# rvp-group/srrg2_laser_slam_2d

Hardware: AMD Instinct MI355X
Metric: scan-to-map alignments/sec (1081-beam vs 100k-pt map, 20 GN iters) (higher is better)
Workload: dtype f32

## Files before the change

### srrg2_laser_slam_2d_amd/csrc/lsm2d_capi_aligner.inc

```
extern "C" uint64_t lsm2d_pair_hash(uint32_t slice, uint32_t fixed_idx, uint32_t moving_idx) {
  const uint32_t a = fixed_idx * 0x9E3779B1u, b = (moving_idx ^ (slice * 0x632BE5ABu)) * 0x85EBCA77u;
  uint32_t lo = a ^ ((b << 13) | (b >> 19)), hi = b ^ ((a << 19) | (a >> 13));
  lo += ((lo << 17) | (lo >> 15)) ^ b;
  hi += ((hi << 11) | (hi >> 21)) ^ a;
  return ((uint64_t) hi << 32) | (uint64_t) lo;
}

extern "C" int32_t lsm2d_stats_capacity(const lsm2d_aligner_params* ap) {
  if (!ap) return 1;
  const long long c = (long long) (ap->max_iterations > 0 ? ap->max_iterations : 0) * (ap->enable_inlier_only_runs ? 2 : 1);
  return (int32_t) (c < 1 ? 1 : (c > 0x7fffffff ? 0x7fffffff : c));
}

struct lsm2d_pending {
  lsm2d_context* ctx = nullptr;
  Lane* lane = nullptr;
  size_t o_pose = 0, o_H = 0, o_status = 0, o_its = 0, o_stats = 0, o_last_pose = 0, o_clock = 0, o_cand = 0;
  int n = 0, stats_stride = 0, n_clock = 0, clock_stride = 0;
  bool zero_copy = false, want_stats = false, want_last_pose = false, stamps = false, timed = false, async = false;
};
static int align_batch_finish(lsm2d_pending& P, float* out_pose, float* out_H, int32_t* out_status, int32_t* out_its, lsm2d_iteration_stats* out_stats, float* out_last_pose);

static constexpr int kEmptyBatch = 0x7e7e7e7e;

// ... 571 lines not shown
    if (zero_copy) { const unsigned long long epoch = ctx->sync_epoch; we = wait_for_statuses(ctx, (const int32_t*) (hs + o_status), n, L.ev_done); ctx->sync_epoch = epoch; }
    else we = hipEventSynchronize(L.ev_done);
    L.busy = false;
    if (ctx->inflight > 0) --ctx->inflight;
    HIPCHK(ctx, we);
  }
  else if (zero_copy) HIPCHK(ctx, wait_for_statuses(ctx, (const int32_t*) (hs + o_status), n));
  else HIPCHK(ctx, stream_sync(ctx));
  ctx->timed_lane = (int) (&L - ctx->lanes); ctx->have_timing = P.timed;
  {
    static_assert(kStatusNotWritten == -1, "the memsets above write 0xFF bytes");
    const int32_t* st = (const int32_t*) (hs + o_status);
    for (int i = 0; i < n; ++i) if (st[i] == kStatusNotWritten) { for (Lane& any : ctx->lanes) any.order_valid = false; return fail(ctx, LSM2D_DEVICE_ERROR, "align_batch: an alignment's workgroup never reported (placement or launch fault)"); }
  }
  memcpy(out_pose, hs + o_pose, sizeof(float) * 3 * (size_t) n);
  if (out_H) memcpy(out_H, hs + o_H, sizeof(float) * 9 * (size_t) n);
  memcpy(out_status, hs + o_status, sizeof(int32_t) * (size_t) n);
  if (out_its) memcpy(out_its, hs + o_its, sizeof(int32_t) * (size_t) n);
  if (out_stats) memcpy(out_stats, hs + o_stats, sizeof(StatsDev) * (size_t) n * (size_t) stats_stride);
  if (out_last_pose) memcpy(out_last_pose, hs + o_last_pose, sizeof(float) * 3 * (size_t) n);
  if (P.want_stats) {
    const uint32_t* cw = (const uint32_t*) (hs + P.o_cand);
    long long its = 0, builds = 0, over = 0;
    for (int i = 0; i < n; ++i) { its += cw[i] & 0xFFFFu; builds += (cw[i] >> 16) & 0xFFu; over += cw[i] >> 24; }
    ctx->last_cand_iterations = (int) std::min(its, (long long) 0x7fffffff); ctx->last_cand_builds = (int) std::min(builds, (long long) 0x7fffffff); ctx->last_cand_overflows = (int) std::min(over, (long long) 0x7fffffff);
  }
  if (stamps) {
    const unsigned long long* ck = (const unsigned long long*) (hs + o_clock);
    std::vector<double> khz; std::vector<unsigned long long> life;
    for (int i = 0; i < n_clock; ++i) if (ck[4 * i + 1] > 0) { khz.push_back((double) ck[4 * i] / (double) ck[4 * i + 1] * 1e5); life.push_back(ck[4 * i + 1] * 10ull); }
    if (const char* dump = getenv("LSM2D_DUMP_STAMPS")) {
      if (FILE* f = fopen(dump, "a")) {
        unsigned long long t0 = ~0ull; for (int i = 0; i < n_clock; ++i) if (ck[4 * i + 1] > 0 && ck[4 * i + 2] < t0) t0 = ck[4 * i + 2];
        fprintf(f, "# launch n=%d stride=%d\n", n, clock_stride);
        for (int i = 0; i < n_clock; ++i)
          fprintf(f, "%d %llu %llu %llu 0x%llx\n", i * clock_stride, ck[4 * i], ck[4 * i + 1], ck[4 * i + 2] - t0, ck[4 * i + 3]);
        fclose(f);
      }
    }
    if (!khz.empty()) {
      std::nth_element(khz.begin(), khz.begin() + khz.size() / 2, khz.end()); ctx->last_clock_khz = (long long) khz[khz.size() / 2];
      std::nth_element(life.begin(), life.begin() + life.size() / 2, life.end()); ctx->last_wg_lifetime_ns = (long long) life[life.size() / 2];
    }
  }
  return LSM2D_SUCCESS;
}

extern "C" int lsm2d_align_batch(lsm2d_context* ctx, const lsm2d_aligner_params* ap, const lsm2d_batch* b, float* out_pose,
                                 float* out_H, int32_t* out_status, int32_t* out_its, lsm2d_iteration_stats* out_stats) {
  return align_batch_impl(ctx, ap, b, out_pose, out_H, out_status, out_its, out_stats, nullptr);
}

extern "C" int lsm2d_align_batch_begin(lsm2d_context* ctx, const lsm2d_aligner_params* ap, const lsm2d_batch* b, int32_t want_stats, lsm2d_pending** out_pending) {
  if (!ctx || !out_pending) return fail(ctx, LSM2D_BAD_ARGUMENT, "align_batch_begin: null argument");
  *out_pending = nullptr;
  lsm2d_pending* P = new (std::nothrow) lsm2d_pending;
  if (!P) return LSM2D_OUT_OF_MEMORY;
  static float dummy_pose; static int32_t dummy_status; static lsm2d_iteration_stats dummy_stats;
  const int rc = align_batch_impl(ctx, ap, b, &dummy_pose, nullptr, &dummy_status, nullptr, want_stats ? &dummy_stats : nullptr, nullptr, nullptr, P);
  if (rc != LSM2D_SUCCESS || !P->ctx) { const bool empty = rc == LSM2D_SUCCESS; delete P; if (!empty) return rc; P = new (std::nothrow) lsm2d_pending; if (!P) return LSM2D_OUT_OF_MEMORY; }
  *out_pending = P;
  return LSM2D_SUCCESS;
}
extern "C" int lsm2d_align_batch_wait(lsm2d_pending* pending, float* out_pose, float* out_H, int32_t* out_status, int32_t* out_its, lsm2d_iteration_stats* out_stats) {
  if (!pending) return LSM2D_BAD_ARGUMENT;
  if (!pending->ctx) { delete pending; return LSM2D_SUCCESS; }
  lsm2d_context* ctx = pending->ctx;
// ... 80 lines not shown
```

### srrg2_laser_slam_2d_amd/csrc/lsm2d_device.h

```cpp
#pragma once
#include <hip/hip_runtime.h>
#include <stdint.h>

namespace lsm2d {

typedef unsigned long long u64;
static constexpr u64 kEmptyCell = ~0ull;

#define LSM2D_DEV __device__ __forceinline__
#define LSM2D_HD  __host__ __device__ inline

struct Iso { float c, s, tx, ty; };

struct ProjK {
  float K00, K01;
  float rmin, rmax;
  float r2lo, r2hi;
  float colsf;
  int   cols;
  int   tiny_ok;
};

LSM2D_HD void sincos_fixed(float x, float& sn, float& cs) {
  const float kf = __builtin_rintf(x * 6.3661974669e-01f);
// ... 259 lines not shown
    const int g = code & 511, t0 = (code >> 9) * B;
    const int nsteps = T_steps - t0 < B ? T_steps - t0 : B;
    const int voff = g * (int) sizeof(float4) + t0 * row_bytes;
    int idx = 2 * (g * T_steps + t0);
    auto load = [&](int soff) {
      const u32x4 w = __builtin_amdgcn_raw_buffer_load_b128(rsrc, voff, soff, 0);
      return make_float4(__uint_as_float(w.x), __uint_as_float(w.y), __uint_as_float(w.z), __uint_as_float(w.w));
    };
    auto pair = [&](const float4& v, int i) {
      project_point_stream<kGuarded>(T, P, v.x, v.y, i, canvas);
      project_point_stream<kGuarded>(T, P, v.z, v.w, i + 1, canvas);
    };
    int t = 0, soff = 0;
    float4 va = load(0);
    for (; t + 2 <= nsteps; t += 2) {
      const float4 vb = load(soff + row_bytes);
      pair(va, idx);
      soff += 2 * row_bytes;
      va = load(soff);
      pair(vb, idx + 2);
      idx += 4;
    }
    if (t < nsteps) pair(va, idx);
  }
}
template <int kStride = 0>
LSM2D_DEV void project_cloud_list(const float4* __restrict__ lane_xy, int T_steps, const Iso& T, const ProjK& P, u64* canvas, int tid, int nthreads,
                                  const uint16_t* units, int n_units, int B) {
  if (P.tiny_ok) project_cloud_list_t<false, kStride>(lane_xy, T_steps, T, P, canvas, tid, nthreads, units, n_units, B);
  else project_cloud_list_t<true, kStride>(lane_xy, T_steps, T, P, canvas, tid, nthreads, units, n_units, B);
}

LSM2D_DEV float cand_depth_margin(float r, float m_t, float tn2 ) { return m_t + __builtin_fmaf(1.0e-6f, r, __builtin_fmaf(2.6e-7f, tn2, 1e-7f)); }
template <bool kGuarded>
LSM2D_DEV int cand_classify(const Iso& T, const ProjK& P, float px, float py, float m_t, float m_th, float tn2, float& r, float& md, int& col) {
  r = 0.0f; md = 0.0f; col = -1;
  if (!(__builtin_fabsf(px) < __builtin_huge_valf() && __builtin_fabsf(py) < __builtin_huge_valf())) return 0;
  float qx, qy;
  xf_point(T, px, py, qx, qy);
  const float r2 = __builtin_fmaf(qx, qx, qy * qy);
  if (!(r2 >= 1e-30f && r2 <= 1e37f)) return 1;
  float y0;
  r = sqrt_rn_seed(r2, y0);
  md = cand_depth_margin(r, m_t, tn2);
  if (r < P.rmin - md || r > P.rmax + md) return 0;
  if (!(md <= 0.25f * r)) return 1;
  const float th = bearing<kGuarded>(qy, qx, r, y0);
  const float u = __builtin_fmaf(P.K00, th, P.K01);
  const float aK = __builtin_fabsf(P.K00);
  const float cs = __builtin_fmaf(aK, __builtin_fmaf(1.06f, md / (r - md), 1.001f * m_th), 4e-3f);
  if ((3.14159274101257324f - __builtin_fabsf(th)) * aK <= cs) return 1;
  if (u < -cs || u > P.colsf + cs) return 0;
  asm("v_cvt_flr_i32_f32 %0, %1" : "=v"(col) : "v"(u));
  if ((unsigned) col >= (unsigned) P.cols) return 1;
  if (!(r >= P.rmin + md && r <= P.rmax - md)) return 1;
  const float f = u - (float) col;
  return (f > cs && 1.0f - f > cs) ? 2 : 1;
}
template <int kStride, class F>
LSM2D_DEV void cand_for_each_pair(const float4* __restrict__ lane_xy, int T_steps, int tid, int nthreads, const uint16_t* units, int n_units, int B, F f) {
  typedef unsigned u32x4 __attribute__((ext_vector_type(4)));
  const unsigned long long pb = reinterpret_cast<unsigned long long>(lane_xy);
  const unsigned pb_hi = (unsigned) __builtin_amdgcn_readfirstlane((int) (pb >> 32));
  const unsigned pb_lo = (unsigned) __builtin_amdgcn_readfirstlane((int) (unsigned) pb);
  float4* ubase = reinterpret_cast<float4*>(((unsigned long long) pb_hi << 32) | (unsigned long long) pb_lo);
  const __amdgpu_buffer_rsrc_t rsrc = __builtin_amdgcn_make_buffer_rsrc(ubase, (short) 0, 0x7fffffff, 0x00020000);
  const int row_bytes = nthreads * (int) sizeof(float4);
  for (int k = tid; k < n_units; k += kStride) {
    const int code = (int) units[k];
    const int g = code & 511, t0 = (code >> 9) * B;
    const int nsteps = T_steps - t0 < B ? T_steps - t0 : B;
    const int voff = g * (int) sizeof(float4) + t0 * row_bytes;
    int idx = 2 * (g * T_steps + t0);
    for (int t = 0; t < nsteps; ++t, idx += 2) {
      const u32x4 w = __builtin_amdgcn_raw_buffer_load_b128(rsrc, voff + t * row_bytes, 0, 0);
      f(__uint_as_float(w.x), __uint_as_float(w.y), __uint_as_float(w.z), __uint_as_float(w.w), idx);
    }
  }
}
template <bool kGuarded, int kStride>
LSM2D_DEV void cand_blockers_t(const float4* __restrict__ lane_xy, int T_steps, const Iso& Tin, const ProjK& Pin, int tid, int nthreads, const uint16_t* units, int n_units, int B,
                               uint32_t* blk, float m_t, float m_th) {
  const Iso T = Tin; const ProjK P = Pin;
  const float tn2 = __builtin_fabsf(T.tx) + __builtin_fabsf(T.ty) + 2.0f * m_t;
  auto one = [&](float px, float py) {
    float r, md; int col;
    if (cand_classify<kGuarded>(T, P, px, py, m_t, m_th, tn2, r, md, col) == 2) atomicMin(&blk[col], __float_as_uint(r + md));
  };
  cand_for_each_pair<kStride>(lane_xy, T_steps, tid, nthreads, units, n_units, B, [&](float ax, float ay, float bx, float by, int) { one(ax, ay); one(bx, by); });
}
template <bool kGuarded, int kStride>
LSM2D_DEV void cand_collect_t(const float4* __restrict__ lane_xy, int T_steps, const Iso& Tin, const ProjK& Pin, int tid, int nthreads, const uint16_t* units, int n_units, int B,
                              const uint32_t* blk, uint32_t* cand, int cap, int* count, float m_t, float m_th) {
  const Iso T = Tin; const ProjK P = Pin;
  const float tn2 = __builtin_fabsf(T.tx) + __builtin_fabsf(T.ty) + 2.0f * m_t;
  auto keeps = [&](float px, float py) -> bool {
    float r, md; int col;
    const int cl = cand_classify<kGuarded>(T, P, px, py, m_t, m_th, tn2, r, md, col);
    if (cl != 2) return cl == 1;
    return !(__uint_as_float(blk[col]) < r - md);
  };
  cand_for_each_pair<kStride>(lane_xy, T_steps, tid, nthreads, units, n_units, B, [&](float ax, float ay, float bx, float by, int idx) {
    const bool k0 = keeps(ax, ay), k1 = keeps(bx, by);
    const u64 b0 = __ballot(k0), b1 = __ballot(k1);
    const u64 act = b0 | b1;
    if (act) {
      const int n0 = __popcll(b0);
      int base = 0;
      if ((int) __builtin_amdgcn_mbcnt_hi((unsigned) (act >> 32), __builtin_amdgcn_mbcnt_lo((unsigned) act, 0u)) == 0 && (k0 || k1)) base = atomicAdd(count, n0 + __popcll(b1));
      base = __builtin_amdgcn_readlane(base, __builtin_amdgcn_readfirstlane(__builtin_ctzll(act)));
      const int p0 = base + (int) __builtin_amdgcn_mbcnt_hi((unsigned) (b0 >> 32), __builtin_amdgcn_mbcnt_lo((unsigned) b0, 0u));
      const int p1 = base + n0 + (int) __builtin_amdgcn_mbcnt_hi((unsigned) (b1 >> 32), __builtin_amdgcn_mbcnt_lo((unsigned) b1, 0u));
      if (k0 && p0 < cap) cand[p0] = (uint32_t) idx;
      if (k1 && p1 < cap) cand[p1] = (uint32_t) (idx + 1);
    }
  });
}
template <bool kGuarded, int kStride>
LSM2D_DEV void project_candidates_t(const float2* __restrict__ mxy, const Iso& Tin, const ProjK& Pin, u64* canvas, int tid, const uint32_t* cand, int n) {
  const Iso T = Tin; ProjK P = Pin;
  asm volatile("" : "+v"(P.K01));
  int k = tid;
  if (k >= n) return;
  int idx = (int) cand[k];
  float2 p = mxy[idx];
  for (; k < n; k += kStride) {
    const int kn = k + kStride;
    const int idn = (int) cand[kn < n ? kn : k];
    const float2 pn = mxy[idn];
    project_point_stream<kGuarded>(T, P, p.x, p.y, idx, canvas);
    idx = idn; p = pn;
  }
}
LSM2D_HD int cand_blocker_words(int cols) { return (cols + 3) & ~3; }
template <int kStride, int kChunks>
LSM2D_DEV void cand_build(const float4* lane_xy, int T_steps, const Iso& T, const ProjK& P, int tid, const uint16_t* units, int n_units, int B, uint32_t* blk, const int* par, int* count) {
  const int cap = __builtin_amdgcn_readfirstlane(par[1]);
  const float m_t = __int_as_float(__builtin_amdgcn_readfirstlane(par[4])), m_th = __int_as_float(__builtin_amdgcn_readfirstlane(par[5]));
  uint32_t* cand = blk + cand_blocker_words(P.cols);
  for (int c = tid; c < P.cols; c += kStride) blk[c] = 0xFFFFFFFFu;
  __syncthreads();
  if (P.tiny_ok) cand_blockers_t<false, kStride>(lane_xy, T_steps, T, P, tid, kChunks, units, n_units, B, blk, m_t, m_th);
  else cand_blockers_t<true, kStride>(lane_xy, T_steps, T, P, tid, kChunks, units, n_units, B, blk, m_t, m_th);
  __syncthreads();
  if (P.tiny_ok) cand_collect_t<false, kStride>(lane_xy, T_steps, T, P, tid, kChunks, units, n_units, B, blk, cand, cap, count, m_t, m_th);
  else cand_collect_t<true, kStride>(lane_xy, T_steps, T, P, tid, kChunks, units, n_units, B, blk, cand, cap, count, m_t, m_th);
}
LSM2D_DEV bool cand_pose_within(const Iso& N, const Iso& L, float m_t, float m_th) {
  if (__float_as_uint(N.c) == __float_as_uint(L.c) && __float_as_uint(N.s) == __float_as_uint(L.s)) {
    const float ex = N.tx - L.tx, ey = N.ty - L.ty;
    return ex * ex + ey * ey <= m_t * m_t * 0.999999f;
  }
  const float cd = N.c * L.c + N.s * L.s, sd = N.s * L.c - N.c * L.s;
  const float dx = N.tx - (cd * L.tx - sd * L.ty), dy = N.ty - (sd * L.tx + cd * L.ty);
  const float lim = m_t - 4e-7f * (__builtin_fabsf(N.tx) + __builtin_fabsf(N.ty) + __builtin_fabsf(L.tx) + __builtin_fabsf(L.ty));
  return cd > 0.5f && __builtin_fabsf(sd) <= m_th - 3e-7f && lim > 0.0f && dx * dx + dy * dy <= lim * lim * 0.999999f;
}

LSM2D_DEV void project_cloud_units(const float4* __restrict__ lane_xy, int T_steps, const Iso& T, const ProjK& P, u64* canvas, int tid, int nthreads,
                                   const uint16_t* surv, int s, int B, int nb) {
  if (P.tiny_ok) project_cloud_units_t<false>(lane_xy, T_steps, T, P, canvas, tid, nthreads, surv, s, B, nb);
  else project_cloud_units_t<true>(lane_xy, T_steps, T, P, canvas, tid, nthreads, surv, s, B, nb);
}

LSM2D_DEV void project_cloud_lanes(const float4* __restrict__ lane_xy, int T_steps, const Iso& T, const ProjK& P,
                                   u64* canvas, int tid, int nthreads) {
  if (P.tiny_ok) project_cloud_lanes_t<false>(lane_xy, T_steps, T, P, canvas, tid, nthreads);
  else project_cloud_lanes_t<true>(lane_xy, T_steps, T, P, canvas, tid, nthreads);
}

struct Accum {
  float h00, h01, h02, h11, h12, h22, b0, b1, b2, chi_in, chi_out;
  int n_in, n_out, n_corr;
};
LSM2D_DEV void accum_zero(Accum& a) {
  a.h00 = a.h01 = a.h02 = a.h11 = a.h12 = a.h22 = a.b0 = a.b1 = a.b2 = a.chi_in = a.chi_out = 0.0f;
  a.n_in = a.n_out = a.n_corr = 0;
// ... 355 lines not shown
```

### srrg2_laser_slam_2d_amd/csrc/lsm2d_k_align.h

```cpp
template <bool kHasProj, bool kHasNN, bool kHasDist, bool kHasKd = false, int kNNMode = 0, bool kSeq = false, int kW = kAlignBlock, bool kCandLists = false>
LSM2D_DEV void align_body(const AlignArgs& A, int a_given = -1) {
  static_assert(kW == kAlignBlock || (kNNMode == 5 && !kSeq && kW % 64 == 0 && kW >= 256 && kW < kAlignBlock), "narrow workgroups: the culled projective stream only");
  __builtin_assume(A.n_slices >= 1 && A.n_slices <= kMaxSlices);
  constexpr bool kNNGlobal = kNNMode == 1, kNNLds = kNNMode == 2;
  constexpr bool kKdAllLds = kNNMode == 3, kKdTop = kNNMode == 4;
  constexpr bool kProjCulled = kNNMode == 5;
  constexpr bool kCand = kCandLists && kProjCulled && !kSeq && kW == kAlignBlock;
  static_assert(kNNMode == 0 || ((kNNMode <= 2) && kHasNN && !kHasProj && !kHasDist && !kHasKd) || ((kNNMode == 3 || kNNMode == 4) && kHasKd && !kHasProj && !kHasDist && !kHasNN) ||
                (kNNMode == 5 && kHasProj && !kHasNN && !kHasDist && !kHasKd), "kNNMode: one finder only");
  extern __shared__ __align__(16) unsigned char smem[];
  u64* mcan = reinterpret_cast<u64*>(smem);
  u64* fcan = mcan + A.cols_max;
  float* red = reinterpret_cast<float*>(fcan + A.fcan_total + ((A.cols_max + A.fcan_total) & 1));
  float2* l_sxy = reinterpret_cast<float2*>(red + (kAlignBlock / 64) * kAccumWords);
  int* l_qc = reinterpret_cast<int*>(red + (kAlignBlock / 64) * kAccumWords);
  uint16_t* l_cst = reinterpret_cast<uint16_t*>(l_sxy + A.nn_lds_points);
  uint16_t* l_sidx = l_cst + ((A.nn_lds_cells + 2) & ~1);
  float4* l_kpl = reinterpret_cast<float4*>(red + (kAlignBlock / 64) * kAccumWords);
  int2* l_klk = reinterpret_cast<int2*>(l_kpl + A.kd_lds_nodes);
  float2* l_kxy = reinterpret_cast<float2*>(l_klk + A.kd_lds_nodes + (A.kd_lds_nodes & 1));
  float2* l_knr = l_kxy + A.kd_lds_points + (A.kd_lds_points & 1);
  __shared__ float s_pose[3];
  __shared__ Iso   s_iso[kMaxSlices];
  __shared__ float s_H[9], s_sum[kAccumWords + 2];
  constexpr int kSumPairs = 13, kSumActive = 14, kSumWords = 15;
  static_assert(kSumWords <= kAccumWords + 2 && kAccumWords + 2 == 16, "s_sum: one word per lane of a row of sixteen");
  __shared__ int   s_done, s_status, s_last_n_in;
  __shared__ float s_prev_chi;
  __shared__ u64 s_dig;
  __shared__ int s_it0;
  __shared__ int s_phase, s_phase_start, s_phase_end;
  __shared__ uint16_t s_surv[kAlignBlock];
  __shared__ int s_wcnt[2 * (kAlignBlock / 64)];
  __shared__ int s_nunits[kMaxSlices], s_rebuild[kMaxSlices];
  __shared__ Iso s_list_iso[kMaxSlices];
  __shared__ Iso s_cand_iso;
  __shared__ int s_cand_n, s_cand_state, s_cand_stat;
  __shared__ int s_cand_par[6];
  uint16_t* l_units = reinterpret_cast<uint16_t*>(smem + A.units_off);
  float* l_rec = reinterpret_cast<float*>(smem + (kSeq ? A.seq_off : 0));
  __shared__ uint32_t s_ring[3 * kFfRing];
  __shared__ int s_ring_n, s_skip;
  __shared__ uint32_t* s_ff_rows;
  __shared__ PriorDev s_prior;

  const int a = a_given >= 0 ? a_given : (A.order ? __builtin_amdgcn_readfirstlane(A.order[blockIdx.x]) : (int) blockIdx.x), tid = threadIdx.x;
  constexpr int nwaves = kW / 64;
  constexpr int kPriorWords = (int) (sizeof(PriorDev) / sizeof(float));
  __shared__ unsigned long long s_clk[2];
#ifdef LSM2D_PHASE_PROBE
  __shared__ unsigned long long s_ph[4];
  if (tid == 0) { s_ph[0] = s_ph[1] = s_ph[2] = 0; s_ph[3] = __builtin_amdgcn_s_memtime(); }
#define LSM2D_PH_STAMP(k) do { if (tid == 0) { const unsigned long long now__ = __builtin_amdgcn_s_memtime(); s_ph[k] += now__ - s_ph[3]; s_ph[3] = now__; } } while (0)
#if LSM2D_PHASE_PROBE + 0 == 2
#define LSM2D_PH(k) LSM2D_PH_STAMP((k) == 0 ? 1 : (k))
#define LSM2D_PH_LISTS() do { } while (0)
#define LSM2D_PH_STREAM() LSM2D_PH_STAMP(0)
#elif LSM2D_PHASE_PROBE + 0 == 3
#define LSM2D_PH(k) LSM2D_PH_STAMP(2)
#define LSM2D_PH_LISTS() LSM2D_PH_STAMP(0)
#define LSM2D_PH_STREAM() LSM2D_PH_STAMP(1)
#elif LSM2D_PHASE_PROBE + 0 == 4
#define LSM2D_PH(k) do { } while (0)
#define LSM2D_PH_LISTS() do { } while (0)
#define LSM2D_PH_STREAM() LSM2D_PH_STAMP(1)
#define LSM2D_PH_SUMS() LSM2D_PH_STAMP(0)
#define LSM2D_PH_TAIL() LSM2D_PH_STAMP(2)
#else
#define LSM2D_PH(k) LSM2D_PH_STAMP(k)
#define LSM2D_PH_LISTS() do { } while (0)
#define LSM2D_PH_STREAM() do { } while (0)
#endif
#else
#define LSM2D_PH(k) do { } while (0)
#define LSM2D_PH_LISTS() do { } while (0)
#define LSM2D_PH_STREAM() do { } while (0)
#endif
#ifndef LSM2D_PH_SUMS
#define LSM2D_PH_SUMS() do { } while (0)
#define LSM2D_PH_TAIL() do { } while (0)
#endif
  if (A.wg_place && tid == 0) A.wg_place[blockIdx.x] = place_key();
  const bool stamp = A.clock_out && tid == 0 && a % A.clock_stride == 0;
  if (stamp) { s_clk[0] = __builtin_amdgcn_s_memtime(); s_clk[1] = __builtin_amdgcn_s_memrealtime(); }
  if (A.prior && tid >= 64 && tid < 64 + kPriorWords)
    ((float*) &s_prior)[tid - 64] = A.inline_n1 ? ((const float*) &A.prior1)[tid - 64] : ((const float*) (A.prior + a))[tid - 64];

  constexpr int kPqRowWords = 5, kPqOccWords = 128 * kPqRowWords;
  __shared__ unsigned s_pqbb[4];
  __shared__ float s_pq[4];
  const bool pq_on = (kHasNN || kHasKd || kHasDist) && A.pq_cull_off > 0;
  uint32_t* l_occ = reinterpret_cast<uint32_t*>(smem + (pq_on ? A.pq_cull_off : 0));
  u64* l_keep = reinterpret_cast<u64*>(l_occ + kPqOccWords);
  auto ordered = [](float f) { const unsigned u = __float_as_uint(f); return (u & 0x80000000u) ? ~u : (u | 0x80000000u); };
  auto unordered = [](unsigned k) { return __uint_as_float((k & 0x80000000u) ? (k & 0x7FFFFFFFu) : ~k); };
  if (pq_on) {
    for (int i = tid; i < kPqOccWords; i += kAlignBlock) l_occ[i] = 0u;
    if (tid < 4) s_pqbb[tid] = tid < 2 ? 0xFFFFFFFFu : 0u;
  }

  if (kHasProj && !kHasNN && !kHasDist && !kHasKd && A.inline_n1)
    for (int s = 0; s < A.n_slices; ++s) if (A.s[s].unpack_src) unpack_fixed_set(A.s[s], tid, kW);
  for (int i = tid; i < A.fcan_total; i += kW) fcan[i] = kEmptyCell;
  for (int i = tid; i < A.cols_max; i += kW) mcan[i] = kEmptyCell;
  auto begin_iteration = [&]() {
    for (int s = 0; s < A.n_slices; ++s) {
      float Xe[3] = {s_pose[0], s_pose[1], s_pose[2]};
      if (A.s[s].has_sensor) compose(A.s[s].cSinv, A.s[s].sSinv, A.s[s].Sinv, s_pose, Xe);
      sincos_fixed(Xe[2], s_iso[s].s, s_iso[s].c); s_iso[s].tx = Xe[0]; s_iso[s].ty = Xe[1];
    }
    float zf = 0.0f; int zi = 0;
    asm volatile("" : "+v"(zf), "+v"(zi));
    for (int k = 0; k < 11; ++k) s_sum[k] = zf;
// ... 144 lines not shown
        ++acc.n_corr; acc.n_in += inl ? 1 : 0; acc.n_out += inl ? 0 : 1;
        seq_have = true;
      };
      int seq_fill = 0;
      auto seq_walk_buffer = [&](int n) {
        if (tid < ((n + 7) & ~7) - n) { float z[kSeqFields]; seq_zero(z); seq_store(l_rec, n + tid, z); }
        __syncthreads();
        if (tid < 64) seq_acc = seq_walk<LSM2D_SEQ_WALK_PRIO != 0>(l_rec, n, tid, seq_acc);
        __syncthreads();
      };
      auto seq_trip = [&](const float (&t)[kSeqFields], int parity ) {
        int n_rec = 0;
        const int pos = block_compact_pos(seq_have, s_wcnt, parity, n_rec, tid, kAlignBlock / 64);
        for (int done = 0; done < n_rec; ) {
          const int room = kSeqHalf - seq_fill, take = n_rec - done < room ? n_rec - done : room;
          if (seq_have && pos >= done && pos < done + take) seq_store(l_rec, seq_fill + pos - done, t);
          seq_fill += take; done += take;
          if (seq_fill == kSeqHalf) { seq_walk_buffer(kSeqHalf); seq_fill = 0; }
        }
        seq_have = false;
      };
      auto seq_flush = [&]() { if (seq_fill > 0) { seq_walk_buffer(seq_fill); seq_fill = 0; } };
      LSM2D_PH(2);
      if (kHasProj && ((!kHasNN && !kHasDist && !kHasKd) || S.finder == LSM2D_FINDER_PROJECTIVE)) {
        {
          const int mc = pick_cloud(S.moving, a);
          if (kProjCulled) {
            const int lane = tid & 63, wave = tid >> 6;
            uint16_t* units = l_units + s * A.units_stride;
            const int Tm = S.moving.lane_T[mc];
            const int nbs = __builtin_amdgcn_readfirstlane(S.moving.block_stride);
            const int B = cull_block_steps(Tm, nbs), nb = (Tm + B - 1) / B;
            const int cst = kCand ? __builtin_amdgcn_readfirstlane(s_cand_state) : 0;
            if (kCand && cst == 1) {
              const float2* mxy = S.moving.xy + S.moving.start[mc];
              const uint32_t* cand = reinterpret_cast<const uint32_t*>(smem + __builtin_amdgcn_readfirstlane(s_cand_par[0])) + cand_blocker_words(S.proj.cols);
              const int n_cand = __builtin_amdgcn_readfirstlane(s_cand_n);
              if (S.proj.tiny_ok) project_candidates_t<false, kW>(mxy, T, S.proj, mcan, tid, cand, n_cand);
              else project_candidates_t<true, kW>(mxy, T, S.proj, mcan, tid, cand, n_cand);
            } else {
            if (__builtin_amdgcn_readfirstlane(s_rebuild[s])) {
              typedef unsigned u32x4 __attribute__((ext_vector_type(4)));
              const float m_t = A.cull_mt, m_th = A.cull_mth;
              const unsigned long long bb = reinterpret_cast<unsigned long long>(S.moving.lane_bounds + (size_t) mc * kAlignBlock);
              float4* bbase = reinterpret_cast<float4*>(((unsigned long long) (unsigned) __builtin_amdgcn_readfirstlane((int) (bb >> 32)) << 32) |
                                                        (unsigned long long) (unsigned) __builtin_amdgcn_readfirstlane((int) (unsigned) bb));
              int n_surv = 0;
              if constexpr (kW == kAlignBlock) {
              const u32x4 bw = __builtin_amdgcn_raw_buffer_load_b128(__builtin_amdgcn_make_buffer_rsrc(bbase, (short) 0, kAlignBlock * 16, 0x00020000), tid * 16, 0, 0);
              const bool keep = chunk_may_matter(T, S.proj, make_float4(__uint_as_float(bw.x), __uint_as_float(bw.y), __uint_as_float(bw.z), 0.0f), fcan + S.fcan_offset, S.point_distance, m_t, m_th);
              const u64 bal = __ballot(keep);
              { int wv = tid >> 6; asm volatile("" : "+v"(wv)); if (lane == 0) s_wcnt[wv] = __popcll(bal); }
              __syncthreads();
              int before = 0;
#pragma unroll
              for (int w = 0; w < nwaves; ++w) { const int cw = s_wcnt[w]; before += w < wave ? cw : 0; n_surv += cw; }
              n_surv = __builtin_amdgcn_readfirstlane(n_surv);
              if (keep) s_surv[before + (int) __builtin_amdgcn_mbcnt_hi((unsigned) (bal >> 32), __builtin_amdgcn_mbcnt_lo((unsigned) bal, 0u))] = (uint16_t) tid;
              __syncthreads();
              } else {
                const __amdgpu_buffer_rsrc_t brs = __builtin_amdgcn_make_buffer_rsrc(bbase, (short) 0, kAlignBlock * 16, 0x00020000);
                int par = 0;
                for (int v0 = 0; v0 < kAlignBlock; v0 += kW, par ^= 1) {
                  const int v = v0 + tid; bool keep = false;
                  if (v < kAlignBlock) {
                    const u32x4 bw = __builtin_amdgcn_raw_buffer_load_b128(brs, v * 16, 0, 0);
                    keep = chunk_may_matter(T, S.proj, make_float4(__uint_as_float(bw.x), __uint_as_float(bw.y), __uint_as_float(bw.z), 0.0f), fcan + S.fcan_offset, S.point_distance, m_t, m_th);
                  }
                  const int pos = block_compact_pos(keep, s_wcnt, par, n_surv, tid, nwaves);
                  if (keep) s_surv[pos] = (uint16_t) v;
                }
                __syncthreads();
              }
              const unsigned long long kb = reinterpret_cast<unsigned long long>(S.moving.block_bounds + (size_t) mc * nbs * kAlignBlock);
              float4* kbase = reinterpret_cast<float4*>(((unsigned long long) (unsigned) __builtin_amdgcn_readfirstlane((int) (kb >> 32)) << 32) |
                                                        (unsigned long long) (unsigned) __builtin_amdgcn_readfirstlane((int) (unsigned) kb));
              const __amdgpu_buffer_rsrc_t krs = __builtin_amdgcn_make_buffer_rsrc(kbase, (short) 0, nbs * kAlignBlock * 16, 0x00020000);
              int n_units = 0, parity = 1, i = tid, blk = 0;
              while (n_surv > 0 && i >= n_surv && blk < nb) { i -= n_surv; ++blk; }
              const int n_tests = nb * n_surv;
              for (int v0 = 0; v0 < n_tests; v0 += kW, parity ^= 1) {
                bool k2 = false; int code = 0;
                if (blk < nb) {
                  const int g = (int) s_surv[i];
                  code = (blk << 9) | g;
                  const u32x4 w4 = __builtin_amdgcn_raw_buffer_load_b128(krs, code * 16, 0, 0);
                  k2 = chunk_may_matter(T, S.proj, make_float4(__uint_as_float(w4.x), __uint_as_float(w4.y), __uint_as_float(w4.z), 0.0f), fcan + S.fcan_offset, S.point_distance, m_t, m_th);
                }
                const int pos = block_compact_pos(k2, s_wcnt, parity, n_units, tid, nwaves);
                if (k2) units[pos] = (uint16_t) code;
                i += kW;
                while (n_surv > 0 && i >= n_surv && blk < nb) { i -= n_surv; ++blk; }
              }
              if (tid == 0) { s_nunits[s] = n_units; s_list_iso[s] = T; }
              __syncthreads();
            }
            LSM2D_PH_LISTS();
            const int n_units = __builtin_amdgcn_readfirstlane(s_nunits[s]);
            if (n_units > 0) project_cloud_list<kW>(S.moving.lane_xy + S.moving.lane_start[mc], Tm, T, S.proj, mcan, tid, kAlignBlock, units, n_units, B);
            if (kCand && cst == 2) {
              uint32_t* blk = reinterpret_cast<uint32_t*>(smem + __builtin_amdgcn_readfirstlane(s_cand_par[0]));
              cand_build<kW, kAlignBlock>(S.moving.lane_xy + S.moving.lane_start[mc], Tm, T, S.proj, tid, units, n_units, B, blk, s_cand_par, &s_cand_n);
            }
            }
          }
          else if (S.moving.lane_xy && S.moving.lane_bounds && A.cull) {
            const int lane = tid & 63, wave = tid >> 6;
            typedef unsigned u32x4 __attribute__((ext_vector_type(4)));
            const unsigned long long bb = reinterpret_cast<unsigned long long>(S.moving.lane_bounds + (size_t) mc * kAlignBlock);
            float4* bbase = reinterpret_cast<float4*>(((unsigned long long) (unsigned) __builtin_amdgcn_readfirstlane((int) (bb >> 32)) << 32) |
                                                      (unsigned long long) (unsigned) __builtin_amdgcn_readfirstlane((int) (unsigned) bb));
            const u32x4 bw = __builtin_amdgcn_raw_buffer_load_b128(__builtin_amdgcn_make_buffer_rsrc(bbase, (short) 0, kAlignBlock * 16, 0x00020000), tid * 16, 0, 0);
            const bool keep = chunk_may_matter(T, S.proj, make_float4(__uint_as_float(bw.x), __uint_as_float(bw.y), __uint_as_float(bw.z), 0.0f), fcan + S.fcan_offset, S.point_distance);
            const u64 bal = __ballot(keep);
            if (lane == 0) s_wcnt[wave] = __popcll(bal);
            __syncthreads();
            int before = 0, n_surv = 0;
#pragma unroll
            for (int w = 0; w < nwaves; ++w) { const int cw = s_wcnt[w]; before += w < wave ? cw : 0; n_surv += cw; }
            if (keep) s_surv[before + (int) __builtin_amdgcn_mbcnt_hi((unsigned) (bal >> 32), __builtin_amdgcn_mbcnt_lo((unsigned) bal, 0u))] = (uint16_t) tid;
            __syncthreads();
            const int Tm = S.moving.lane_T[mc];
            const int B = cull_block_steps(Tm), nb = (Tm + B - 1) / B;
            if (n_surv > 0) project_cloud_units(S.moving.lane_xy + S.moving.lane_start[mc], Tm, T, S.proj, mcan, tid, kAlignBlock, s_surv, n_surv, B, nb);
          }
          else if (S.moving.lane_xy) project_cloud_lanes(S.moving.lane_xy + S.moving.lane_start[mc], S.moving.lane_T[mc], T, S.proj, mcan, tid, kAlignBlock);
          else project_cloud(S.moving.xy + S.moving.start[mc], S.moving.count[mc], T, S.proj, mcan, tid, kAlignBlock);
        }
        __syncthreads();
        LSM2D_PH_STREAM();
        const int mbase = S.moving.start[pick_cloud(S.moving, a)], fbase = S.fixed.start[pick_cloud(S.fixed, a)];
        const float2* mn = S.moving.nrm + mbase; const float2* mp = S.moving.xy + mbase;
        const float2* fnr = S.fixed.nrm + fbase; const float2* fpp = S.fixed.xy + fbase;
        const float4* maos = S.moving.aos ? S.moving.aos + mbase : nullptr;
        const float4* faos = S.fixed.aos ? S.fixed.aos + fbase : nullptr;
// ... 247 lines not shown
        const int n_corr_s = __builtin_amdgcn_readlane(vi, 13);
        const bool act = n_corr_s > S.min_corr;
        float tot = cur;
        if (act || ln == kSumPairs) tot = ln < 11 ? cur + v : __int_as_float(__float_as_int(cur) + (ln == kSumPairs ? n_corr_s : (ln == kSumActive ? 1 : vi)));
        if (ln < kSumWords) s_sum[ln] = tot;
      }
      LSM2D_PH(1);
      if (kHasNN || kHasDist || kHasKd) __syncthreads();
    }
    if (tid < 64) {
      int ln = tid; asm volatile("" : "+v"(ln));
      const int l16 = ln & (kFfRing - 1);
      static_assert(kFfRing == 16 && kMaxSlices == 4, "lane masks below");
      const float p0 = s_pose[0], p1 = s_pose[1], p2 = s_pose[2];
      const int n = s_ring_n, phase_end = s_phase_end;
      uint32_t* const ffw = s_ff_rows;
      const Iso iso0 = s_iso[0], Ll = s_list_iso[ln & 3];
      const uint32_t e0 = s_ring[3 * l16], e1 = s_ring[3 * l16 + 1], e2 = s_ring[3 * l16 + 2];
      const float tot = s_sum[l16];
#define LSM2D_RL_F(x, k) __int_as_float(__builtin_amdgcn_readlane(__float_as_int(x), k))
      const int hk = ln - 32;
      const bool h_lane = (unsigned) hk < 9u;
      const int n_corr = __builtin_amdgcn_readlane(__float_as_int(tot), kSumPairs), active = __builtin_amdgcn_readlane(__float_as_int(tot), kSumActive);
      const int n_in = __builtin_amdgcn_readlane(__float_as_int(tot), 11);
      const float chi_in = LSM2D_RL_F(tot, 9), chi_out = LSM2D_RL_F(tot, 10);
      if (ln == 0) s_last_n_in = n_in;
      int skip = 0;
      if (A.out_stats) {
        static_assert(sizeof(StatsDev) == 28, "seven words: n_corr n_in n_out chi_in chi_out dig_lo dig_hi");
        int n_out = __builtin_amdgcn_readlane(__float_as_int(tot), 12); float chi_o = chi_out;
#ifdef LSM2D_DEBUG_UNITS
        if (kProjCulled) { n_out = s_nunits[0]; chi_o = (float) s_rebuild[0]; }
#endif
        const u64 dg = s_dig;
        const int w = ln == 0 ? n_corr : ln == 1 ? n_in : ln == 2 ? n_out : ln == 3 ? __float_as_int(chi_in) : ln == 4 ? __float_as_int(chi_o) : ln == 5 ? (int) (uint32_t) dg : (int) (uint32_t) (dg >> 32);
        if (ln < 7) reinterpret_cast<int32_t*>(A.out_stats + (size_t) a * A.stats_stride + it)[ln] = w;
      }
      bool done = false;
      float np0 = 0.0f, np1 = 0.0f, np2 = 0.0f;
      if (!active) { if (ln == 0) { s_status = LSM2D_NOT_ENOUGH_CORRESPONDENCES; s_done = 1; } done = true; }
      else {
        float x0 = LSM2D_RL_F(tot, 0), x1 = LSM2D_RL_F(tot, 1), x2 = LSM2D_RL_F(tot, 2), x3 = LSM2D_RL_F(tot, 3), x4 = LSM2D_RL_F(tot, 4), x5 = LSM2D_RL_F(tot, 5),
              x6 = LSM2D_RL_F(tot, 6), x7 = LSM2D_RL_F(tot, 7), x8 = LSM2D_RL_F(tot, 8);
        float Hq = (hk == 0) ? x0 : (hk == 1 || hk == 3) ? x1 : (hk == 2 || hk == 6) ? x2 : (hk == 4) ? x3 : (hk == 5 || hk == 7) ? x4 : x5;
        if (A.prior) {
          const int pr = h_lane ? hk / 3 : (int) ((0x210211000ull >> (4 * l16)) & 15), pc = h_lane ? hk - 3 * (hk / 3) : (int) ((0x333221210ull >> (4 * l16)) & 15);
          float P = 0.0f;
          if (ln < 9 || h_lane) P = prior_term_lane_call(s_prior, p0, p1, p2, pr, pc);
          Hq += P;
          const float tp = tot + P;
          x0 = LSM2D_RL_F(tp, 0); x1 = LSM2D_RL_F(tp, 1); x2 = LSM2D_RL_F(tp, 2); x3 = LSM2D_RL_F(tp, 3); x4 = LSM2D_RL_F(tp, 4); x5 = LSM2D_RL_F(tp, 5);
          x6 = LSM2D_RL_F(tp, 6); x7 = LSM2D_RL_F(tp, 7); x8 = LSM2D_RL_F(tp, 8);
        }
        if (h_lane) s_H[hk] = Hq;
        if (ff_on) {
          if (ln < 3) s_ring[3 * (n & (kFfRing - 1)) + ln] = __float_as_uint(ln == 0 ? p0 : (ln == 1 ? p1 : p2));
          if (ln == 0) s_ring_n = n + 1;
        }
        float dmp = A.damping;
        asm volatile("" : "+v"(dmp));
        float dx, dy, dth;
        const bool ok = solve_flat(x0, x1, x2, x3, x4, x5, x6, x7, x8, dmp, dx, dy, dth);
        if (!ok) { if (ln == 0) { s_status = LSM2D_SINGULAR_H; s_done = 1; } done = true; }
        else {
          float sn = iso0.s, cs = iso0.c;
          if (A.s[0].has_sensor) sincos_fixed(p2, sn, cs);
          np0 = __builtin_fmaf(cs, dx, __builtin_fmaf(-sn, dy, p0));
// ... 71 lines not shown
          Iso N; sincos_fixed(Xe[2], N.s, N.c); N.tx = Xe[0]; N.ty = Xe[1];
          const Iso cur0 = s_iso[0];
          s_iso[ln] = N;
          if (kProjCulled) {
            const float cd = N.c * Ll.c + N.s * Ll.s, sd = N.s * Ll.c - N.c * Ll.s;
            const float ddx = N.tx - (cd * Ll.tx - sd * Ll.ty), ddy = N.ty - (sd * Ll.tx + cd * Ll.ty);
            const int rb = (A.cull_keep && cd > 0.5f && __builtin_fabsf(sd) <= A.cull_mth && ddx * ddx + ddy * ddy <= A.cull_mt2) ? 0 : 1;
            s_rebuild[ln] = rb;
            if (kCand && s_cand_par[0] > 0 && ln == 0) {
              int st = s_cand_state, stat = s_cand_stat;
              const int n_built = s_cand_n, cap = s_cand_par[1], first_it = s_cand_par[2], max_builds = s_cand_par[3];
              const float mt = __int_as_float(s_cand_par[4]), mth = __int_as_float(s_cand_par[5]);
              Iso Lc = s_cand_iso;
              if (st == 2) {
                const bool fits = n_built <= cap;
                int over = fits ? 0 : 1; asm volatile("" : "+v"(over));
                stat += 0x10000 + (over << 24);
                st = fits ? 1 : 0;
                if (fits) { Lc = cur0; s_cand_iso = cur0; }
              }
              const bool serves = st == 1 && !rb && cand_pose_within(N, Lc, mt, mth);
              const bool build = !serves && it + 1 >= first_it && ((stat >> 16) & 0xFF) < max_builds && (stat >> 24) == 0;
              if (serves && (stat & 0xFFFF) != 0xFFFF) ++stat;
              s_cand_state = serves ? 1 : (build ? 2 : 0);
              s_cand_stat = stat;
              if (build) s_cand_n = 0;
            }
          }
        }
        int zi = 0; asm volatile("" : "+v"(zi));
        if (ln < kSumWords) s_sum[ln] = __int_as_float(zi);
        if (ln == 0) s_dig = (u64) (unsigned) zi;
        if (A.out_last_pose && ln < 3) A.out_last_pose[3 * a + ln] = ln == 0 ? np0 : (ln == 1 ? np1 : np2);
      }
    }
    LSM2D_PH(2);
    LSM2D_PH_TAIL();
    __syncthreads();
    if (ff_on) it += __builtin_amdgcn_readfirstlane(s_skip);
    if (s_done) { ++it; break; }
  }
  if (tid == 0) {
    int st = s_status;
    if (st == LSM2D_RUNNING) st = (A.max_it > 0 && s_last_n_in < A.min_inliers) ? LSM2D_NOT_ENOUGH_INLIERS : LSM2D_SUCCESS;
    A.out_pose[3 * a + 0] = s_pose[0]; A.out_pose[3 * a + 1] = s_pose[1]; A.out_pose[3 * a + 2] = s_pose[2];
    if (A.out_H) for (int k = 0; k < 9; ++k) A.out_H[9 * a + k] = s_H[k];
    if (A.out_its) A.out_its[a] = it;
    if (kCand && A.cand_out) A.cand_out[a] = s_cand_stat;
    if (stamp) {
      unsigned long long* co = A.clock_out + 4 * (a / A.clock_stride);
      co[0] = __builtin_amdgcn_s_memtime() - s_clk[0];
      co[1] = __builtin_amdgcn_s_memrealtime() - s_clk[1];
      co[2] = s_clk[1];
#ifdef LSM2D_PHASE_PROBE
      co[1] = s_ph[0]; co[2] = s_ph[1]; co[3] = s_ph[2];
      if (A.host_polls) { __threadfence_system(); __hip_atomic_store(&A.out_status[a], st, __ATOMIC_RELEASE, __HIP_MEMORY_SCOPE_SYSTEM); } else A.out_status[a] = st;
      return;
#endif
      co[3] = (unsigned long long) __builtin_amdgcn_s_getreg((31 << 11) | (0 << 6) | 4) |
              ((unsigned long long) __builtin_amdgcn_s_getreg((31 << 11) | (0 << 6) | 20) << 32);
    }
    if (A.host_polls) { __threadfence_system(); __hip_atomic_store(&A.out_status[a], st, __ATOMIC_RELEASE, __HIP_MEMORY_SCOPE_SYSTEM); }
    else A.out_status[a] = st;
  }
}
#ifndef LSM2D_MIXED_MIN_WAVES
// ... 42 lines not shown
```

Baseline: 2.145 million.

## Fuse candidate blocker computation into the canvas projection pass

On candidate-build iterations, the moving cloud was projected onto the canvas and then traversed a second time to compute per-column blocker depths. The blocker atomicMin is now issued inside the projection pass, reusing the computed range, bearing and column, so one full pass over the moving points and its polar transform is removed. Classification logic is split into a polar helper shared by both paths. It also adds phase-probe macros, a debug digest option, and build-stat accounting in the non-active branch, and projection now runs after the blocker clear and barrier on build iterations.

```diff
diff --git a/srrg2_laser_slam_2d_amd/csrc/lsm2d_capi_aligner.inc b/srrg2_laser_slam_2d_amd/csrc/lsm2d_capi_aligner.inc
--- a/srrg2_laser_slam_2d_amd/csrc/lsm2d_capi_aligner.inc
+++ b/srrg2_laser_slam_2d_amd/csrc/lsm2d_capi_aligner.inc
@@ -627,7 +627,7 @@
     if (const char* dump = getenv("LSM2D_DUMP_STAMPS")) {
       if (FILE* f = fopen(dump, "a")) {
         unsigned long long t0 = ~0ull; for (int i = 0; i < n_clock; ++i) if (ck[4 * i + 1] > 0 && ck[4 * i + 2] < t0) t0 = ck[4 * i + 2];
-        fprintf(f, "# launch n=%d stride=%d\n", n, clock_stride);
+        fprintf(f, "# launch n=%d stride=%d t0=%llu\n", n, clock_stride, t0);
         for (int i = 0; i < n_clock; ++i)
           fprintf(f, "%d %llu %llu %llu 0x%llx\n", i * clock_stride, ck[4 * i], ck[4 * i + 1], ck[4 * i + 2] - t0, ck[4 * i + 3]);
         fclose(f);
diff --git a/srrg2_laser_slam_2d_amd/csrc/lsm2d_device.h b/srrg2_laser_slam_2d_amd/csrc/lsm2d_device.h
--- a/srrg2_laser_slam_2d_amd/csrc/lsm2d_device.h
+++ b/srrg2_laser_slam_2d_amd/csrc/lsm2d_device.h
@@ -315,6 +315,19 @@
 }
 
 LSM2D_DEV float cand_depth_margin(float r, float m_t, float tn2 ) { return m_t + __builtin_fmaf(1.0e-6f, r, __builtin_fmaf(2.6e-7f, tn2, 1e-7f)); }
+LSM2D_DEV int cand_classify_polar(const ProjK& P, float r, float th, float u, int col , float m_t, float m_th, float tn2, float& md) {
+  md = cand_depth_margin(r, m_t, tn2);
+  if (r < P.rmin - md || r > P.rmax + md) return 0;
+  if (!(md <= 0.25f * r)) return 1;
+  const float aK = __builtin_fabsf(P.K00);
+  const float cs = __builtin_fmaf(aK, __builtin_fmaf(1.06f, md / (r - md), 1.001f * m_th), 4e-3f);
+  if ((3.14159274101257324f - __builtin_fabsf(th)) * aK <= cs) return 1;
+  if (u < -cs || u > P.colsf + cs) return 0;
+  if ((unsigned) col >= (unsigned) P.cols) return 1;
+  if (!(r >= P.rmin + md && r <= P.rmax - md)) return 1;
+  const float f = u - (float) col;
+  return (f > cs && 1.0f - f > cs) ? 2 : 1;
+}
 template <bool kGuarded>
 LSM2D_DEV int cand_classify(const Iso& T, const ProjK& P, float px, float py, float m_t, float m_th, float tn2, float& r, float& md, int& col) {
   r = 0.0f; md = 0.0f; col = -1;
@@ -325,20 +338,72 @@
   if (!(r2 >= 1e-30f && r2 <= 1e37f)) return 1;
   float y0;
   r = sqrt_rn_seed(r2, y0);
-  md = cand_depth_margin(r, m_t, tn2);
-  if (r < P.rmin - md || r > P.rmax + md) return 0;
-  if (!(md <= 0.25f * r)) return 1;
   const float th = bearing<kGuarded>(qy, qx, r, y0);
   const float u = __builtin_fmaf(P.K00, th, P.K01);
-  const float aK = __builtin_fabsf(P.K00);
-  const float cs = __builtin_fmaf(aK, __builtin_fmaf(1.06f, md / (r - md), 1.001f * m_th), 4e-3f);
-  if ((3.14159274101257324f - __builtin_fabsf(th)) * aK <= cs) return 1;
-  if (u < -cs || u > P.colsf + cs) return 0;
   asm("v_cvt_flr_i32_f32 %0, %1" : "=v"(col) : "v"(u));
-  if ((unsigned) col >= (unsigned) P.cols) return 1;
-  if (!(r >= P.rmin + md && r <= P.rmax - md)) return 1;
-  const float f = u - (float) col;
-  return (f > cs && 1.0f - f > cs) ? 2 : 1;
+  const int cl = cand_classify_polar(P, r, th, u, col, m_t, m_th, tn2, md);
+  if ((unsigned) col >= (unsigned) P.cols) col = -1;
+  return cl;
+}
+template <bool kGuarded>
+LSM2D_DEV void project_point_stream_blk(const Iso& T, const ProjK& P, float px, float py, int idx, u64* canvas, uint32_t* blk, const int* par) {
+  float qx, qy;
+  xf_point(T, px, py, qx, qy);
+  const float r2 = __builtin_fmaf(qx, qx, qy * qy);
+  if (r2 >= P.r2lo && r2 <= P.r2hi) {
+    float y0;
+    const float r  = sqrt_rn_seed(r2, y0);
+    const float th = bearing<kGuarded>(qy, qx, r, y0);
+    const float u  = __builtin_fmaf(P.K00, th, P.K01);
+    int col;
+    asm("v_cvt_flr_i32_f32 %0, %1" : "=v"(col) : "v"(u));
+    if ((unsigned) col < (unsigned) P.cols) {
+      atomicMin(&canvas[col], ((u64) __float_as_uint(r) << 32) | (u64) (uint32_t) idx);
+      const float m_t = __int_as_float(par[4]), m_th = __int_as_float(par[5]);
+      const float tn2 = __builtin_fabsf(T.tx) + __builtin_fabsf(T.ty) + 2.0f * m_t;
+      float md;
+      if (cand_classify_polar(P, r, th, u, col, m_t, m_th, tn2, md) == 2) atomicMin(&blk[col], __float_as_uint(r + md));
+    }
+  }
+}
+template <bool kGuarded, int kStride>
+LSM2D_DEV void project_cloud_list_blk_t(const float4* __restrict__ lane_xy, int T_steps, const Iso& Tin, const ProjK& Pin, u64* canvas, int tid, int nthreads,
+                                        const uint16_t* units, int n_units, int B, uint32_t* blk, const int* par) {
+  const Iso T = Tin; ProjK P = Pin;
+  asm volatile("" : "+v"(P.K01));
+  typedef unsigned u32x4 __attribute__((ext_vector_type(4)));
+  const unsigned long long pb = reinterpret_cast<unsigned long long>(lane_xy);
+  const unsigned pb_hi = (unsigned) __builtin_amdgcn_readfirstlane((int) (pb >> 32));
+  const unsigned pb_lo = (unsigned) __builtin_amdgcn_readfirstlane((int) (unsigned) pb);
+  float4* ubase = reinterpret_cast<float4*>(((unsigned long long) pb_hi << 32) | (unsigned long long) pb_lo);
+  const __amdgpu_buffer_rsrc_t rsrc = __builtin_amdgcn_make_buffer_rsrc(ubase, (short) 0, 0x7fffffff, 0x00020000);
+  const int row_bytes = nthreads * (int) sizeof(float4);
+  for (int k = tid; k < n_units; k += kStride) {
+    const int code = (int) units[k];
+    const int g = code & 511, t0 = (code >> 9) * B;
+    const int nsteps = T_steps - t0 < B ? T_steps - t0 : B;
+    const int voff = g * (int) sizeof(float4) + t0 * row_bytes;
+    int idx = 2 * (g * T_steps + t0);
+    auto load = [&](int soff) {
+      const u32x4 w = __builtin_amdgcn_raw_buffer_load_b128(rsrc, voff, soff, 0);
+      return make_float4(__uint_as_float(w.x), __uint_as_float(w.y), __uint_as_float(w.z), __uint_as_float(w.w));
+    };
+    auto pair = [&](const float4& v, int i) {
+      project_point_stream_blk<kGuarded>(T, P, v.x, v.y, i, canvas, blk, par);
+      project_point_stream_blk<kGuarded>(T, P, v.z, v.w, i + 1, canvas, blk, par);
+    };
+    int t = 0, soff = 0;
+    float4 va = load(0);
+    for (; t + 2 <= nsteps; t += 2) {
+      const float4 vb = load(soff + row_bytes);
+      pair(va, idx);
+      soff += 2 * row_bytes;
+      va = load(soff);
+      pair(vb, idx + 2);
+      idx += 4;
+    }
+    if (t < nsteps) pair(va, idx);
+  }
 }
 template <int kStride, class F>
 LSM2D_DEV void cand_for_each_pair(const float4* __restrict__ lane_xy, int T_steps, int tid, int nthreads, const uint16_t* units, int n_units, int B, F f) {
@@ -360,17 +425,6 @@
       f(__uint_as_float(w.x), __uint_as_float(w.y), __uint_as_float(w.z), __uint_as_float(w.w), idx);
     }
   }
-}
-template <bool kGuarded, int kStride>
-LSM2D_DEV void cand_blockers_t(const float4* __restrict__ lane_xy, int T_steps, const Iso& Tin, const ProjK& Pin, int tid, int nthreads, const uint16_t* units, int n_units, int B,
-                               uint32_t* blk, float m_t, float m_th) {
-  const Iso T = Tin; const ProjK P = Pin;
-  const float tn2 = __builtin_fabsf(T.tx) + __builtin_fabsf(T.ty) + 2.0f * m_t;
-  auto one = [&](float px, float py) {
-    float r, md; int col;
-    if (cand_classify<kGuarded>(T, P, px, py, m_t, m_th, tn2, r, md, col) == 2) atomicMin(&blk[col], __float_as_uint(r + md));
-  };
-  cand_for_each_pair<kStride>(lane_xy, T_steps, tid, nthreads, units, n_units, B, [&](float ax, float ay, float bx, float by, int) { one(ax, ay); one(bx, by); });
 }
 template <bool kGuarded, int kStride>
 LSM2D_DEV void cand_collect_t(const float4* __restrict__ lane_xy, int T_steps, const Iso& Tin, const ProjK& Pin, int tid, int nthreads, const uint16_t* units, int n_units, int B,
@@ -416,16 +470,19 @@
   }
 }
 LSM2D_HD int cand_blocker_words(int cols) { return (cols + 3) & ~3; }
+template <int kStride>
+LSM2D_DEV void cand_clear_blockers(const ProjK& P, int tid, uint32_t* blk) { for (int c = tid; c < P.cols; c += kStride) blk[c] = 0xFFFFFFFFu; }
+template <int kStride>
+LSM2D_DEV void project_cloud_list_blk(const float4* __restrict__ lane_xy, int T_steps, const Iso& T, const ProjK& P, u64* canvas, int tid, int nthreads,
+                                      const uint16_t* units, int n_units, int B, uint32_t* blk, const int* par) {
+  if (P.tiny_ok) project_cloud_list_blk_t<false, kStride>(lane_xy, T_steps, T, P, canvas, tid, nthreads, units, n_units, B, blk, par);
+  else project_cloud_list_blk_t<true, kStride>(lane_xy, T_steps, T, P, canvas, tid, nthreads, units, n_units, B, blk, par);
+}
 template <int kStride, int kChunks>
-LSM2D_DEV void cand_build(const float4* lane_xy, int T_steps, const Iso& T, const ProjK& P, int tid, const uint16_t* units, int n_units, int B, uint32_t* blk, const int* par, int* count) {
+LSM2D_DEV void cand_collect(const float4* lane_xy, int T_steps, const Iso& T, const ProjK& P, int tid, const uint16_t* units, int n_units, int B, uint32_t* blk, const int* par, int* count) {
   const int cap = __builtin_amdgcn_readfirstlane(par[1]);
   const float m_t = __int_as_float(__builtin_amdgcn_readfirstlane(par[4])), m_th = __int_as_float(__builtin_amdgcn_readfirstlane(par[5]));
   uint32_t* cand = blk + cand_blocker_words(P.cols);
-  for (int c = tid; c < P.cols; c += kStride) blk[c] = 0xFFFFFFFFu;
-  __syncthreads();
-  if (P.tiny_ok) cand_blockers_t<false, kStride>(lane_xy, T_steps, T, P, tid, kChunks, units, n_units, B, blk, m_t, m_th);
-  else cand_blockers_t<true, kStride>(lane_xy, T_steps, T, P, tid, kChunks, units, n_units, B, blk, m_t, m_th);
-  __syncthreads();
   if (P.tiny_ok) cand_collect_t<false, kStride>(lane_xy, T_steps, T, P, tid, kChunks, units, n_units, B, blk, cand, cap, count, m_t, m_th);
   else cand_collect_t<true, kStride>(lane_xy, T_steps, T, P, tid, kChunks, units, n_units, B, blk, cand, cap, count, m_t, m_th);
 }
diff --git a/srrg2_laser_slam_2d_amd/csrc/lsm2d_k_align.h b/srrg2_laser_slam_2d_amd/csrc/lsm2d_k_align.h
--- a/srrg2_laser_slam_2d_amd/csrc/lsm2d_k_align.h
+++ b/srrg2_laser_slam_2d_amd/csrc/lsm2d_k_align.h
@@ -52,6 +52,7 @@
   __shared__ unsigned long long s_ph[4];
   if (tid == 0) { s_ph[0] = s_ph[1] = s_ph[2] = 0; s_ph[3] = __builtin_amdgcn_s_memtime(); }
 #define LSM2D_PH_STAMP(k) do { if (tid == 0) { const unsigned long long now__ = __builtin_amdgcn_s_memtime(); s_ph[k] += now__ - s_ph[3]; s_ph[3] = now__; } } while (0)
+#define LSM2D_PH_SKIP() do { if (tid == 0) s_ph[3] = __builtin_amdgcn_s_memtime(); } while (0)
 #if LSM2D_PHASE_PROBE + 0 == 2
 #define LSM2D_PH(k) LSM2D_PH_STAMP((k) == 0 ? 1 : (k))
 #define LSM2D_PH_LISTS() do { } while (0)
@@ -66,6 +67,16 @@
 #define LSM2D_PH_STREAM() LSM2D_PH_STAMP(1)
 #define LSM2D_PH_SUMS() LSM2D_PH_STAMP(0)
 #define LSM2D_PH_TAIL() LSM2D_PH_STAMP(2)
+#elif LSM2D_PHASE_PROBE + 0 == 5
+#define LSM2D_PH(k) do { } while (0)
+#define LSM2D_PH_LISTS() LSM2D_PH_SKIP()
+#define LSM2D_PH_STREAM() do { } while (0)
+#define LSM2D_PH_CAND(k) do { if ((k) >= 0 && (k) <= 2) LSM2D_PH_STAMP((k) & 3); else LSM2D_PH_SKIP(); } while (0)
+#elif LSM2D_PHASE_PROBE + 0 == 6
+#define LSM2D_PH(k) do { } while (0)
+#define LSM2D_PH_LISTS() LSM2D_PH_STAMP(2)
+#define LSM2D_PH_STREAM() do { } while (0)
+#define LSM2D_PH_CAND(k) do { if ((k) == 3) LSM2D_PH_STAMP(0); else if ((k) == 4) LSM2D_PH_STAMP(1); else LSM2D_PH_SKIP(); } while (0)
 #else
 #define LSM2D_PH(k) LSM2D_PH_STAMP(k)
 #define LSM2D_PH_LISTS() do { } while (0)
@@ -79,6 +90,9 @@
 #ifndef LSM2D_PH_SUMS
 #define LSM2D_PH_SUMS() do { } while (0)
 #define LSM2D_PH_TAIL() do { } while (0)
+#endif
+#ifndef LSM2D_PH_CAND
+#define LSM2D_PH_CAND(k) do { } while (0)
 #endif
   if (A.wg_place && tid == 0) A.wg_place[blockIdx.x] = place_key();
   const bool stamp = A.clock_out && tid == 0 && a % A.clock_stride == 0;
@@ -289,12 +303,14 @@
             const int nbs = __builtin_amdgcn_readfirstlane(S.moving.block_stride);
             const int B = cull_block_steps(Tm, nbs), nb = (Tm + B - 1) / B;
             const int cst = kCand ? __builtin_amdgcn_readfirstlane(s_cand_state) : 0;
+            LSM2D_PH_CAND(-1);
             if (kCand && cst == 1) {
               const float2* mxy = S.moving.xy + S.moving.start[mc];
               const uint32_t* cand = reinterpret_cast<const uint32_t*>(smem + __builtin_amdgcn_readfirstlane(s_cand_par[0])) + cand_blocker_words(S.proj.cols);
               const int n_cand = __builtin_amdgcn_readfirstlane(s_cand_n);
               if (S.proj.tiny_ok) project_candidates_t<false, kW>(mxy, T, S.proj, mcan, tid, cand, n_cand);
               else project_candidates_t<true, kW>(mxy, T, S.proj, mcan, tid, cand, n_cand);
+              LSM2D_PH_CAND(2);
             } else {
             if (__builtin_amdgcn_readfirstlane(s_rebuild[s])) {
               typedef unsigned u32x4 __attribute__((ext_vector_type(4)));
@@ -354,10 +370,18 @@
             }
             LSM2D_PH_LISTS();
             const int n_units = __builtin_amdgcn_readfirstlane(s_nunits[s]);
-            if (n_units > 0) project_cloud_list<kW>(S.moving.lane_xy + S.moving.lane_start[mc], Tm, T, S.proj, mcan, tid, kAlignBlock, units, n_units, B);
             if (kCand && cst == 2) {
               uint32_t* blk = reinterpret_cast<uint32_t*>(smem + __builtin_amdgcn_readfirstlane(s_cand_par[0]));
-              cand_build<kW, kAlignBlock>(S.moving.lane_xy + S.moving.lane_start[mc], Tm, T, S.proj, tid, units, n_units, B, blk, s_cand_par, &s_cand_n);
+              cand_clear_blockers<kW>(S.proj, tid, blk);
+              __syncthreads();
+              if (n_units > 0) project_cloud_list_blk<kW>(S.moving.lane_xy + S.moving.lane_start[mc], Tm, T, S.proj, mcan, tid, kAlignBlock, units, n_units, B, blk, s_cand_par);
+              __syncthreads();
+              LSM2D_PH_CAND(1);
+              cand_collect<kW, kAlignBlock>(S.moving.lane_xy + S.moving.lane_start[mc], Tm, T, S.proj, tid, units, n_units, B, blk, s_cand_par, &s_cand_n);
+              LSM2D_PH_CAND(4);
+            } else {
+              if (n_units > 0) project_cloud_list<kW>(S.moving.lane_xy + S.moving.lane_start[mc], Tm, T, S.proj, mcan, tid, kAlignBlock, units, n_units, B);
+              LSM2D_PH_CAND(0);
             }
             }
           }
@@ -671,7 +695,10 @@
 #ifdef LSM2D_DEBUG_UNITS
         if (kProjCulled) { n_out = s_nunits[0]; chi_o = (float) s_rebuild[0]; }
 #endif
-        const u64 dg = s_dig;
+        u64 dg = s_dig;
+#ifdef LSM2D_DEBUG_CAND
+        if (kCand) dg = ((u64) (unsigned) s_cand_n << 32) | (u64) (unsigned) s_cand_state;
+#endif
         const int w = ln == 0 ? n_corr : ln == 1 ? n_in : ln == 2 ? n_out : ln == 3 ? __float_as_int(chi_in) : ln == 4 ? __float_as_int(chi_o) : ln == 5 ? (int) (uint32_t) dg : (int) (uint32_t) (dg >> 32);
         if (ln < 7) reinterpret_cast<int32_t*>(A.out_stats + (size_t) a * A.stats_stride + it)[ln] = w;
       }
@@ -809,6 +836,10 @@
         if (ln < kSumWords) s_sum[ln] = __int_as_float(zi);
         if (ln == 0) s_dig = (u64) (unsigned) zi;
         if (A.out_last_pose && ln < 3) A.out_last_pose[3 * a + ln] = ln == 0 ? np0 : (ln == 1 ? np1 : np2);
+      } else if (kCand && ln == 0 && s_cand_par[0] > 0) {
+        int built = s_cand_state == 2 ? 1 : 0, over = s_cand_n > s_cand_par[1] ? 1 : 0;
+        asm volatile("" : "+v"(built), "+v"(over));
+        s_cand_stat += (built << 16) + ((built & over) << 24);
       }
     }
     LSM2D_PH(2);
```

Result: faster. 2.313 million, median of 6 (+7.8%).
